# leodd/Lifted-Hybrid-Variational-Inference

Measured on AMD Instinct MI355X. Metric: lbp_sweeps_per_sec_10M_edge_hybrid_mrf, higher is better.
Workload: dtype f64

## Files before the change

### include/lhvi.h

```cpp
#ifndef LHVI_H
#define LHVI_H

#include <stddef.h>
#include <stdint.h>

#ifdef __cplusplus
extern "C" {
#endif

#define LHVI_ABI_VERSION 27
#define LHVI_MAX_ARITY 6

#define LHVI_OK 0
#define LHVI_E_ARG (-1)
#define LHVI_E_LAUNCH (-2)
#define LHVI_E_UNSUPPORTED (-3)
#define LHVI_E_NODEVICE (-4)
#define LHVI_E_NOT_PD (-5)

#define LHVI_POT_GENERIC 0
#define LHVI_POT_TABLE 1
#define LHVI_POT_GAUSSIAN 2
#define LHVI_POT_QUADRATIC 3
#define LHVI_POT_HYBRID_QUADRATIC 4
#define LHVI_POT_LINEAR_GAUSSIAN 5
#define LHVI_POT_X2 6
#define LHVI_POT_XY 7
#define LHVI_POT_MLN 8
#define LHVI_POT_MLN_HARD 9
#define LHVI_POT_IMAGE_NODE 10
#define LHVI_POT_IMAGE_EDGE 11

typedef struct lhvi_graph {
    int32_t V, F, E, nnz;
    const int32_t* fac_ptr;
    const int32_t* edge_var;
    const int32_t* edge_fac;
    const int32_t* edge_canon;
    const int32_t* var_ptr;
    const int32_t* var_edge;
    const double* edge_count;
    const int32_t* fac_pot;
    const double* var_value;
// ... 41 lines not shown
    const int32_t* seg;
    int32_t n_seg;
} lhvi_gabp_plan_t;
size_t lhvi_gabp_pull_workspace_bytes(const lhvi_graph_t* g);
int lhvi_gabp_pull(const lhvi_graph_t* g, const lhvi_pots_t* pots, const lhvi_gabp_plan_t* plan, const double* v_prev,
                   double* v_next, int first, void* stream);
int lhvi_gabp_run_pull(const lhvi_graph_t* g, const lhvi_pots_t* pots, const lhvi_gabp_plan_t* plan, double* f2v, double* v2f,
                       int iterations, void* ws, size_t ws_bytes, void* stream);

int lhvi_gabp_graph_create(const lhvi_graph_t* g, const lhvi_pots_t* pots, const lhvi_gabp_plan_t* plan, double* f2v, double* v2f,
                           double* mu_var, int iterations, void* ws, size_t ws_bytes, void** handle_out);
int lhvi_gabp_graph_launch(void* handle, void* stream);
int lhvi_gabp_graph_destroy(void* handle);

int lhvi_gabp_marginals(const lhvi_graph_t* g, const double* f2v, double* mu_var, void* stream);

size_t lhvi_log_likelihood_workspace_bytes(const lhvi_graph_t* g);
int lhvi_log_likelihood(const lhvi_graph_t* g, const lhvi_pots_t* pots, const double* x, double* out, void* ws, size_t ws_bytes,
                        void* stream);


#define LHVI_PBP_EP 1u
#define LHVI_PBP_EPBP_DISCRETE 2u
#define LHVI_PBP_SKIP_TERMS 16u
#define LHVI_PBP_LEAVE_ROOM 256u
#define LHVI_PBP_CQ 512u
#define LHVI_PBP_BOUNDARY_TOTALS 2048u
#define LHVI_PBP_NO_UNIQ 4096u
#define LHVI_PBP_V2F_RECORDS 8192u
#define LHVI_PBP_WIDE_PAIRS 16384u
#define LHVI_PBP_SHARE_CUS 32768u
#define LHVI_PBP_NO_GRID 128u
#define LHVI_PBP_FUSED_RECORDS16 131072u
#define LHVI_PBP_F2V_HEAVY 262144u
#define LHVI_PBP_F2V_SMALL 524288u
#define LHVI_PBP_F2V_PAIR 1048576u
#define LHVI_PBP_F2V_FAST 2097152u
#define LHVI_PBP_F2V_CQ 4194304u
#define LHVI_PBP_F2V_GENERIC 8388608u
#define LHVI_PBP_F2V_ALL (LHVI_PBP_F2V_HEAVY | LHVI_PBP_F2V_SMALL | LHVI_PBP_F2V_PAIR | LHVI_PBP_F2V_FAST | LHVI_PBP_F2V_CQ | LHVI_PBP_F2V_GENERIC)
#define LHVI_PBP_POW2_GROUPS 65536u

typedef struct lhvi_pbp {
    int32_t n;
    int32_t T;
    uint32_t flags;
    double var_threshold;
    double max_log_value;
    const double* particles;
    const double* old_particles;
    const int32_t* np;
    const uint8_t* uniq;
    const double* q;
    const int32_t* fast_edges;
    int32_t n_fast;
    const int32_t* generic_edges;
    int32_t n_generic;
    int32_t generic_pts_log2;
    const void* fast_desc;
    const void* heavy_desc;
    int32_t n_heavy;
    const void* light_desc;
    int32_t n_light;
    const int32_t* bslot;
    const int32_t* brow_ptr;
    const int64_t* brow_off;
// ... 400 lines not shown
```

### lifted-hybrid-variational-inference_amd/csrc/pbp.hip

```cpp
#include "common.hpp"
#include "potential.hpp"
#include "fastmath.hpp"
#include "cq.hpp"
#include "gk21.hpp"

namespace lhvi {

__device__ __forceinline__ double wave_sum(double v) { return dpp_wave_reduce(v, SumOp()); }
__device__ __forceinline__ double wave_max(double v) { return dpp_wave_reduce(v, MaxOp()); }
__device__ __forceinline__ int wave_sum_i(int v) {
#pragma unroll
    for (int off = 32; off > 0; off >>= 1) v += __shfl_xor(v, off);
    return v;
}

constexpr double PAD_LOG_TERM = -6.0e5;

__host__ __device__ __forceinline__ int var_first(const lhvi_pbp_t& s) { return s.var_hi > s.var_lo ? s.var_lo : 0; }
__host__ __device__ __forceinline__ int var_limit(const lhvi_graph_t& g, const lhvi_pbp_t& s) { return s.var_hi > s.var_lo ? s.var_hi : g.V; }

__device__ __forceinline__ double norm_pdf_std(double x, double mu, double sig) {
    const double u = (x - mu) / sig;
    return exp(-u * u * 0.5) / (2.506628274631 * sig);
}
// ... 197 lines not shown
    for (; k < deg; k += NW) {
        const int e = g.var_edge[lo + k];
        const double m = valid ? f2v[(int64_t)e * S + lane] : 0.0;
        acc += lifted ? m * g.edge_count[e] : m;
    }
    part[wid][lane] = acc;
    __syncthreads();
    double total = 0.0;
#pragma unroll
    for (int w = 0; w < NW; ++w) total += part[w][lane];
    const int d = g.var_dom[v];
    const double mu = s.q[2 * v], sd = sqrt_pos(s.q[2 * v + 1]), rsd = rcp_newton(sd);
    const double log_norm = log_pos(2.506628274631 * sd);
    const double x = valid ? s.particles[(int64_t)v * n + lane] : 0.0;
    const bool uq = valid && s.uniq[(int64_t)v * n + lane];
    const double logw = valid ? log_importance(g, s, v, d, x, mu, rsd, log_norm) : 0.0;
    const double rcnt = rcp_newton((double)__builtin_popcountll(__ballot(uq)));
    for (k = wid; k < deg; k += NW) {
        const int e = g.var_edge[lo + k];
        const double m = valid ? f2v[(int64_t)e * S + lane] : 0.0;
        const double res = (total - m) + logw;
        const double mean = wave_sum(uq ? res : 0.0) * rcnt;
        double shift = mean;
        if (__ballot(uq && (res - mean > s.max_log_value))) shift = wave_max(uq ? res : -__builtin_huge_val()) - s.max_log_value;
        if (valid) {
            v2f[(int64_t)e * n + lane] = res - shift;
            const int64_t halo = HALO ? s.halo_off[e] : -1;
            if (HALO && halo >= 0) s.halo_buf[halo + lane] = res - shift;
        }
    }
}

template <bool HALO>
__global__ void __launch_bounds__(BLOCK) pbp_v2f_narrow_kernel(lhvi_graph_t g, lhvi_pbp_t s, const double* __restrict__ f2v,
                                                              double* __restrict__ v2f) {
    const int lane = threadIdx.x & 63;
    const int64_t slot = ((int64_t)blockIdx.x * (BLOCK / WAVE) + (threadIdx.x >> 6)) * 16 + (lane >> 2);
    const int j = lane & 3;
    const int v = slot < s.n_v2f_narrow ? s.v2f_narrow[slot] : -1;
    const int n = s.n, S = s.n + s.T;
    const bool on = v >= 0 && is_hidden(g.var_value[v]);
    const int np = on ? s.np[v] : 0;
    const bool valid = j < np;
    const int lo = on ? g.var_ptr[v] : 0, deg = on ? g.var_ptr[v + 1] - lo : 0;
    const bool lifted = g.edge_count != nullptr;
    double total = 0.0;
    for (int k = 0; k < deg; ++k) {
        const int e = g.var_edge[lo + k];
        const double m = valid ? f2v[(int64_t)e * S + j] : 0.0;
        total += lifted ? m * g.edge_count[e] : m;
    }
    double logw = 0.0;
    bool uq = false;
    if (valid) {
        const int d = g.var_dom[v];
        const double sd = sqrt_pos(s.q[2 * v + 1]);
        logw = log_importance(g, s, v, d, s.particles[(int64_t)v * n + j], s.q[2 * v], rcp_newton(sd), log_pos(2.506628274631 * sd));
        uq = s.uniq[(int64_t)v * n + j] != 0;
    }
    auto quad_sum = [](double x) { x += dpp_move<0xb1>(x); return x + dpp_move<0x4e>(x); };
    auto quad_max = [](double x) { x = fmax(x, dpp_move<0xb1>(x)); return fmax(x, dpp_move<0x4e>(x)); };
    const double rcnt = rcp_newton(fmax(quad_sum(uq ? 1.0 : 0.0), 1.0));
    int maxdeg = deg;
#pragma unroll
    for (int off = 32; off > 0; off >>= 1) maxdeg = max(maxdeg, __shfl_xor(maxdeg, off));
    for (int k = 0; k < maxdeg; ++k) {
        const bool live = k < deg;
        const int e = live ? g.var_edge[lo + k] : 0;
        const double m = (live && valid) ? f2v[(int64_t)e * S + j] : 0.0;
        const double res = (total - m) + logw;
        const double mean = quad_sum(uq ? res : 0.0) * rcnt;
        const double mx = quad_max(uq ? res : -__builtin_huge_val());
        const double shift = (mx - mean > s.max_log_value) ? mx - s.max_log_value : mean;
        if (live && valid) {
            v2f[(int64_t)e * n + j] = res - shift;
            const int64_t halo = HALO ? s.halo_off[e] : -1;
            if (HALO && halo >= 0) s.halo_buf[halo + j] = res - shift;
        }
    }
}

template <int W, bool HALO>
__global__ void __launch_bounds__(BLOCK) pbp_v2f_packed_kernel(lhvi_graph_t g, lhvi_pbp_t s, const double* __restrict__ f2v,
                                                              double* __restrict__ v2f, const int32_t* __restrict__ list, int count) {
    constexpr int G = WAVE / W;
    const int lane = threadIdx.x & 63;
    const int64_t slot = ((int64_t)blockIdx.x * (BLOCK / WAVE) + (threadIdx.x >> 6)) * G + lane / W;
    const int j = lane % W;
    const int v = slot < count ? list[slot] : -1;
    const int n = s.n, S = s.n + s.T;
    const bool on = v >= 0 && is_hidden(g.var_value[v]);
    const int np = on ? s.np[v] : 0;
    const bool valid = j < np;
    const int lo = on ? g.var_ptr[v] : 0, deg = on ? g.var_ptr[v + 1] - lo : 0;
    const bool lifted = g.edge_count != nullptr;
    double total = 0.0;
    for (int k = 0; k < deg; ++k) {
        const int e = g.var_edge[lo + k];
        const double m = valid ? f2v[(int64_t)e * S + j] : 0.0;
        total += lifted ? m * g.edge_count[e] : m;
    }
    double logw = 0.0;
    bool uq = false;
    if (valid) {
        const int d = g.var_dom[v];
        const double sd = sqrt_pos(s.q[2 * v + 1]);
        logw = log_importance(g, s, v, d, s.particles[(int64_t)v * n + j], s.q[2 * v], rcp_newton(sd), log_pos(2.506628274631 * sd));
        uq = s.uniq[(int64_t)v * n + j] != 0;
    }
    auto group_sum = [&](double x) { return W == 16 ? dpp_move<0x15F>(dpp_row_reduce(x, SumOp())) : dpp_half_reduce(x, SumOp(), lane); };
    auto group_max = [&](double x) { return W == 16 ? dpp_row_reduce(x, MaxOp()) : dpp_half_reduce(x, MaxOp(), lane); };
    const uint64_t mine = (W == 16 ? 0xffffull : 0xffffffffull) << (lane / W * W);
    const double rcnt = rcp_newton(fmax((double)__builtin_popcountll(__ballot(uq) & mine), 1.0));
// ... 2124 lines not shown
                while (todo) {
                    const int k = __builtin_ctzll(todo);
                    const int klo = __builtin_amdgcn_readlane(xlo[h], k), khi = __builtin_amdgcn_readlane(xhi[h], k);
                    const uint64_t same = __ballot(xlo[h] == klo && xhi[h] == khi) & live;
                    dp |= same & (same - 1);
                    todo &= ~same;
                }
            }
            const int u = (lane < cn) && !((dp >> lane) & 1);
            if (lane < n) uniq[(int64_t)vv[h] * n + lane] = (uint8_t)u;
        }
    }
}

#ifndef LHVI_FUSED_WAVES
#define LHVI_FUSED_WAVES 4
#endif
constexpr int FUSED_CH = 8;
#ifndef LHVI_FUSED_NB
#define LHVI_FUSED_NB 2
#endif
#ifndef LHVI_FUSED64_WAVES
#define LHVI_FUSED64_WAVES 8
#endif
#ifndef LHVI_FUSED64_CH
#define LHVI_FUSED64_CH 4
#endif
#ifndef LHVI_FUSED64_PRE
#define LHVI_FUSED64_PRE 1
#endif
#ifndef LHVI_FUSED64_EARLY
#define LHVI_FUSED64_EARLY 1
#endif
#ifndef LHVI_FUSED64_LATE_TABLE
#define LHVI_FUSED64_LATE_TABLE 1
#endif
constexpr int FUSED_CH64 = LHVI_FUSED64_CH;
constexpr int FUSED64_HASH_BITS = 12;
template <int W, int PW, bool EP, bool R16>
__global__ void __launch_bounds__(BLOCK) __attribute__((amdgpu_waves_per_eu(W == 64 ? (PW == 32 || EP ? LHVI_FUSED_WAVES : LHVI_FUSED64_WAVES) : LHVI_FUSED_WAVES, 8)))
pbp_var_fused_kernel(lhvi_graph_t g, lhvi_pbp_t s, const double* __restrict__ f2v, double* __restrict__ v2f, double* __restrict__ eta,
                     double* __restrict__ q, const int64_t* __restrict__ gid, uint64_t seed, uint32_t iteration,
                     double* __restrict__ out, uint8_t* __restrict__ uniq, const int32_t* __restrict__ list, int count) {
    __shared__ LogRec sh_log[LOG_TAB_N];
    __shared__ uint8_t sh_owner[W == 64 ? (BLOCK / WAVE) << FUSED64_HASH_BITS : 1];
    constexpr bool LATE_TABLE = W == 64 && LHVI_FUSED64_LATE_TABLE != 0;
    double tab_inv = 0.0, tab_log = 0.0;
    if constexpr (LATE_TABLE) {
        if (threadIdx.x < LOG_TAB_N) { tab_inv = LOG_TAB[2 * threadIdx.x]; tab_log = LOG_TAB[2 * threadIdx.x + 1]; }
    } else {
        load_log_table(sh_log);
        __syncthreads();
    }
    constexpr int G = WAVE / W, SL = W / PW;
    const int lane = threadIdx.x & 63;
    const int wave = W == 64 ? __builtin_amdgcn_readfirstlane(threadIdx.x >> 6) : (int)(threadIdx.x >> 6);
    const int64_t slot = ((int64_t)blockIdx.x * (BLOCK / WAVE) + wave) * G + lane / W;
    const int j = lane % W;
    const bool on = slot < count;
    const int32_t* rec = list + (R16 ? 16 : 8) * (on ? slot : 0);
    int4 ra, rb;
    int2 rc = make_int2(0, 0);
    int e_rec = 0;
    if (R16) {
        const int4* r4 = reinterpret_cast<const int4*>(rec);
        ra = r4[0]; rb = r4[1]; rc = reinterpret_cast<const int2*>(rec)[4];
        e_rec = rec[10 + min(lane % W, 5)];
    } else {
        ra = make_int4(rec[0], rec[1], rec[2], rec[3]); rb = make_int4(rec[4], rec[5], rec[6], rec[7]);
    }
    const int v = on ? ra.x : 0;
    const int deg = on ? ra.y : 0, gb = ra.z, T = on ? ra.w : 0;
    const double dlo = __hiloint2double(rb.y, rb.x), dhi = __hiloint2double(rb.w, rb.z);
    const int n = s.n, S = s.n + s.T;
    const int np = on ? (R16 ? rc.x : s.np[v]) : 0;
    const bool valid = j < np;
    const int lo = on ? (R16 ? rc.y : g.var_ptr[v]) : 0;
    const bool lifted = g.edge_count != nullptr;
    const double q0 = on ? s.q[2 * v] : 0.0, q1 = on ? s.q[2 * v + 1] : 1.0;
    int maxdeg = deg;
#pragma unroll
    for (int off = 32; off >= W; off >>= 1) maxdeg = max(maxdeg, __shfl_xor(maxdeg, off));
    constexpr int CH = W == 64 ? FUSED_CH64 : FUSED_CH;
    static_assert(W >= CH && CH % SL == 0, "lane j of a group holds edge j of the chunk");
    static_assert(W < 64 || R16, "the one-variable-per-wavefront form reads sixteen-word records");
    const int first_lane = lane / W * W;
    const int nch = (maxdeg + CH - 1) / CH;
    int my_e = 0, held = -1;
    auto hold_chunk = [&](int c) {
        if (c == held) return;
// ... 648 lines not shown
    hipLaunchKernelGGL(pbp_belief_kernel, dim3(grid_for((int64_t)nq * npts)), dim3(BLOCK), 0, as_stream(stream), *g, *pots, *s,
                       v2f, nq, qvar, npts, x, out);
    return check_launch();
}

int lhvi_pbp_map_brent(const lhvi_graph_t* g, const lhvi_pots_t* pots, const lhvi_pbp_t* s, const double* v2f, int64_t nq,
                       const int32_t* row_var, const int64_t* qptr, const int32_t* qedge, const double* qmult, double xtol,
                       int32_t maxfun, double* xout, double* fout, int32_t* nfev, void* stream) {
    if (int rc = validate_pbp(g, s)) return rc;
    if (!pots || !v2f || nq < 0 || maxfun < 1 || !(xtol > 0.0)) return LHVI_E_ARG;
    if (nq == 0) return LHVI_OK;
    if (!row_var || !xout || !g->dom_lo || !g->dom_hi || !g->dom_val) return LHVI_E_ARG;
    if (qptr && (!qedge || !qmult)) return LHVI_E_ARG;
    QueryRows rows{row_var, qptr, qedge, qmult};
    hipLaunchKernelGGL(pbp_map_brent_kernel, dim3(grid_for(nq)), dim3(BLOCK), 0, as_stream(stream), *g, *pots, *s, v2f, nq, rows,
                       row_var, xtol / 3.0, maxfun, xout, fout, nfev);
    return check_launch();
}

int lhvi_pbp_var_fused(const lhvi_graph_t* g, const lhvi_pbp_t* s, const double* f2v, double* v2f, double* eta, double* q,
                       const int64_t* var_gid, uint64_t seed, uint32_t iteration, double* particles_out, uint8_t* uniq_out,
                       const int32_t* desc, int32_t n16, int32_t n32_t32, int32_t n32_t64, void* stream) {
    if (int rc = validate_pbp(g, s)) return rc;
    if (!f2v || !v2f || !eta || !q || !particles_out || !uniq_out || !s->uniq || !s->q || !g->dom_lo || !g->dom_hi || !g->dom_val) return LHVI_E_ARG;
    if (n16 < 0 || n32_t32 < 0 || n32_t64 < 0 || s->n > 32 || s->bslot || s->var_hi > s->var_lo || particles_out == s->particles) return LHVI_E_ARG;
    if ((int64_t)n16 + n32_t32 + n32_t64 == 0) return LHVI_OK;
    if (!desc) return LHVI_E_ARG;
    hipStream_t st = as_stream(stream);
    const bool ep = (s->flags & LHVI_PBP_EP) != 0;
#define LHVI_FUSED(W, PW, list, cnt)                                                                                                  \
    if ((cnt) > 0) {                                                                                                                  \
        const dim3 grid(grid_for(((int64_t)(cnt) + WAVE / (W) - 1) / (WAVE / (W)) * WAVE));                                          \
        if (ep && r16) hipLaunchKernelGGL((pbp_var_fused_kernel<W, PW, true, true>), grid, dim3(BLOCK), 0, st, *g, *s, f2v, v2f, eta, q, var_gid, \
                                   seed, iteration, particles_out, uniq_out, list, cnt);                                             \
        else if (ep) hipLaunchKernelGGL((pbp_var_fused_kernel<W, PW, true, false>), grid, dim3(BLOCK), 0, st, *g, *s, f2v, v2f, eta, q, var_gid, \
                                   seed, iteration, particles_out, uniq_out, list, cnt);                                             \
        else if (r16) hipLaunchKernelGGL((pbp_var_fused_kernel<W, PW, false, true>), grid, dim3(BLOCK), 0, st, *g, *s, f2v, v2f, eta, q, var_gid,   \
                                seed, iteration, particles_out, uniq_out, list, cnt);                                                \
        else hipLaunchKernelGGL((pbp_var_fused_kernel<W, PW, false, false>), grid, dim3(BLOCK), 0, st, *g, *s, f2v, v2f, eta, q, var_gid,   \
                                seed, iteration, particles_out, uniq_out, list, cnt);                                                \
    }
    const bool r16 = (s->flags & LHVI_PBP_FUSED_RECORDS16) != 0;
    const int64_t rw = r16 ? 16 : 8;
    LHVI_FUSED(16, 16, desc, n16)
    LHVI_FUSED(32, 16, desc + rw * (int64_t)n16, n32_t32)
    LHVI_FUSED(32, 32, desc + rw * ((int64_t)n16 + n32_t32), n32_t64)
#undef LHVI_FUSED
    return check_launch();
}

int lhvi_pbp_var_fused64(const lhvi_graph_t* g, const lhvi_pbp_t* s, const double* f2v, double* v2f, double* eta, double* q,
                         const int64_t* var_gid, uint64_t seed, uint32_t iteration, double* particles_out, uint8_t* uniq_out,
                         const int32_t* desc, int32_t n64_t32, int32_t n64_t64, void* stream) {
    if (int rc = validate_pbp(g, s)) return rc;
    if (!f2v || !v2f || !eta || !q || !particles_out || !uniq_out || !s->uniq || !s->q || !g->dom_lo || !g->dom_hi || !g->dom_val) return LHVI_E_ARG;
    if (n64_t32 < 0 || n64_t64 < 0 || s->n <= 32 || s->n > 64 || s->bslot || s->var_hi > s->var_lo || particles_out == s->particles) return LHVI_E_ARG;
    if ((int64_t)n64_t32 + n64_t64 == 0) return LHVI_OK;
    if (!desc) return LHVI_E_ARG;
    hipStream_t st = as_stream(stream);
    const bool ep = (s->flags & LHVI_PBP_EP) != 0;
#define LHVI_FUSED64(PW, list, cnt)                                                                                                   \
    if ((cnt) > 0) {                                                                                                                  \
        const dim3 grid(grid_for((int64_t)(cnt) * WAVE));                                                                             \
        if (ep) hipLaunchKernelGGL((pbp_var_fused_kernel<64, PW, true, true>), grid, dim3(BLOCK), 0, st, *g, *s, f2v, v2f, eta, q, var_gid, \
                                   seed, iteration, particles_out, uniq_out, list, cnt);                                             \
        else hipLaunchKernelGGL((pbp_var_fused_kernel<64, PW, false, true>), grid, dim3(BLOCK), 0, st, *g, *s, f2v, v2f, eta, q, var_gid,   \
                                seed, iteration, particles_out, uniq_out, list, cnt);                                                \
    }
    LHVI_FUSED64(16, desc, n64_t32)
    LHVI_FUSED64(32, desc + 16 * (int64_t)n64_t32, n64_t64)
#undef LHVI_FUSED64
    return check_launch();
}

int lhvi_pbp_quad(const lhvi_graph_t* g, const lhvi_pots_t* pots, const lhvi_pbp_t* s, const double* v2f, int64_t nq,
                  const int32_t* row_var, const int64_t* qptr, const int32_t* qedge, const double* qmult, const double* lo,
                  const double* hi, double epsabs, double epsrel, double* z, double* abserr, int32_t* status, void* stream) {
    if (int rc = validate_pbp(g, s)) return rc;
    if (!pots || !v2f || nq < 0 || !(epsabs >= 0.0) || !(epsrel >= 0.0)) return LHVI_E_ARG;
    if (nq == 0) return LHVI_OK;
    if (!row_var || !lo || !hi || !z) return LHVI_E_ARG;
    if (qptr && (!qedge || !qmult)) return LHVI_E_ARG;
    QueryRows rows{row_var, qptr, qedge, qmult};
    hipLaunchKernelGGL(pbp_quad_kernel, dim3(grid_for(nq)), dim3(BLOCK), 0, as_stream(stream), *g, *pots, *s, v2f, nq, rows, row_var,
                       lo, hi, epsabs, epsrel, z, abserr, status);
    return check_launch();
}

int lhvi_pbp_kl(const lhvi_graph_t* g, const lhvi_pots_t* pots, const lhvi_pbp_t* s, const double* v2f, int64_t nq,
                const int32_t* row_var, const int64_t* qptr, const int32_t* qedge, const double* qmult, const double* logz,
                int32_t Kp, const double* wp, const double* mup, const double* varp, const double* a, const double* b,
                double epsabs, double epsrel, double* kl, double* abserr, int32_t* status, int32_t* neval, void* stream) {
    if (int rc = validate_pbp(g, s)) return rc;
    if (!pots || !v2f || nq < 1 || nq > 0x7fffffff || Kp < 1 || !(epsabs >= 0.0) || !(epsrel >= 0.0)) return LHVI_E_ARG;
    if (!row_var || !logz || !wp || !mup || !varp || !a || !b || !kl) return LHVI_E_ARG;
    if (g->V < 1 || !g->dom_lo || !g->dom_hi || !g->dom_val) return LHVI_E_ARG;
    if (qptr && (!qedge || !qmult)) return LHVI_E_ARG;
    QueryRows rows{row_var, qptr, qedge, qmult};
    hipLaunchKernelGGL(pbp_kl_kernel, dim3((unsigned)nq), dim3(WAVE), 0, as_stream(stream), *g, *pots, *s, v2f, rows, row_var, logz,
                       Kp, wp, mup, varp, a, b, epsabs, epsrel, kl, abserr, status, neval);
// ... 5 lines not shown
```

### lifted-hybrid-variational-inference_amd/lhvi/_abi.py

```python
from __future__ import annotations

import ctypes as C
import os

import numpy as np

_HERE = os.path.dirname(os.path.abspath(__file__))
LIB_PATH = os.environ.get('LHVI_LIB') or os.path.join(os.path.dirname(_HERE), 'csrc', 'liblhvi.so')

c_i32p = C.c_void_p
c_f64p = C.c_void_p


class LhviError(RuntimeError):
    pass


class GraphStruct(C.Structure):
    _fields_ = [
        ('V', C.c_int32), ('F', C.c_int32), ('E', C.c_int32), ('nnz', C.c_int32),
        ('fac_ptr', C.c_void_p), ('edge_var', C.c_void_p), ('edge_fac', C.c_void_p), ('edge_canon', C.c_void_p),
        ('var_ptr', C.c_void_p), ('var_edge', C.c_void_p), ('edge_count', C.c_void_p), ('fac_pot', C.c_void_p),
        ('var_value', C.c_void_p), ('var_dom', C.c_void_p), ('var_mult', C.c_void_p), ('fac_mult', C.c_void_p),
        ('D', C.c_int32),
# ... 35 lines not shown
        ('halo_off', C.c_void_p), ('halo_buf', C.c_void_p),
    ]


class ViStruct(C.Structure):
    _fields_ = [
        ('K', C.c_int32), ('T', C.c_int32), ('Dmax', C.c_int32), ('quirks', C.c_int32),
        ('gh_x', C.c_void_p), ('gh_w', C.c_void_p), ('w', C.c_void_p), ('eta_c', C.c_void_p), ('eta_d', C.c_void_p),
        ('obs_var', C.c_void_p), ('var_N', C.c_void_p),
        ('fac_list', C.c_void_p), ('n_cc', C.c_int32), ('n_grp3', C.c_int32), ('n_grp6', C.c_int32), ('n_rest3', C.c_int32),
        ('n_rest6', C.c_int32), ('n_tiny', C.c_int32), ('tiny_par_words', C.c_int32), ('edge_axis', C.c_void_p),
    ]


class ViOptStruct(C.Structure):
    _fields_ = [(n, C.c_void_p) for n in ('w_tau', 'w', 'eta_c', 'tau_d', 'eta_d', 'm_w', 's_w', 'm_c', 's_c', 'm_d', 's_d',
                                          'g_w', 'g_c', 'g_d', 'fe')] + \
               [(n, C.c_double) for n in ('lr', 'b1', 'b2', 'eps', 'var_min')] + [('t', C.c_int32)]


PBP_EP = 1
PBP_EPBP_DISCRETE = 2
PBP_SKIP_TERMS = 16
PBP_NO_GRID = 128
PBP_LEAVE_ROOM = 256
PBP_BOUNDARY_TOTALS = 2048
PBP_CQ = 512
PBP_NO_UNIQ = 4096
PBP_V2F_RECORDS = 8192
PBP_WIDE_PAIRS = 16384
PBP_SHARE_CUS = 32768
PBP_POW2_GROUPS = 65536
PBP_FUSED_RECORDS16 = 131072
PBP_F2V_HEAVY = 262144
PBP_F2V_SMALL = 524288
PBP_F2V_PAIR = 1048576
PBP_F2V_FAST = 2097152
PBP_F2V_CQ = 4194304
PBP_F2V_GENERIC = 8388608
PBP_F2V_ALL = PBP_F2V_HEAVY | PBP_F2V_SMALL | PBP_F2V_PAIR | PBP_F2V_FAST | PBP_F2V_CQ | PBP_F2V_GENERIC
ABI_VERSION = 27
PBP_DESC_BYTES = 128
COLOR_HASH, COLOR_SORT = 0, 1
HUB_DEGREE = 64
VI_GROUP_SLOTS, VI_GROUP_COMP, VI_TINY_NODES, VI_TINY_K, VI_TINY_PAR = 24, 48, 32, 2, 3072

class MwsStruct(C.Structure):
    _fields_ = [('T', C.c_int32), ('max_flips', C.c_int32), ('epsilon', C.c_double), ('noise_std', C.c_double),
                ('seed', C.c_uint64), ('try_id', C.c_void_p), ('disc', C.c_void_p), ('n_disc', C.c_int32),
                ('num', C.c_void_p), ('n_num', C.c_int32), ('fac_class', C.c_void_p), ('x', C.c_void_p), ('best_x', C.c_void_p),
                ('cur_score', C.c_void_p), ('best_score', C.c_void_p), ('status', C.c_void_p), ('err_flip', C.c_void_p),
                ('rec_score', C.c_void_p), ('rec_zero', C.c_void_p), ('rec_ticks', C.c_void_p)] + \
               [(n, C.c_void_p) for n in ('rp_init', 'rp_clause', 'rp_walk', 'rp_walk_k', 'rp_noise', 'rp_post', 'out_score',
                                          'out_unsat', 'out_winner', 'out_accept', 'out_val')]


class ExactStruct(C.Structure):
    _fields_ = [('Nd', C.c_int32), ('Nc', C.c_int32), ('M', C.c_int64), ('dstates', C.c_void_p), ('dstride', C.c_void_p),
                ('n_quad', C.c_int32), ('quad_ptr', C.c_void_p), ('quad_desc', C.c_void_p), ('quad_par', C.c_void_p),
                ('n_tab', C.c_int32), ('tab_ptr', C.c_void_p), ('tab_desc', C.c_void_p), ('tab_par', C.c_void_p)]


class GibbsStruct(C.Structure):
    _fields_ = [('ex', ExactStruct), ('dstate_off', C.c_void_p), ('vt_ptr', C.c_void_p), ('vt_fac', C.c_void_p),
                ('vh_ptr', C.c_void_p), ('vh_fac', C.c_void_p), ('n_hyb', C.c_int32), ('hyb_quad', C.c_void_p),
                ('hyb_off', C.c_void_p), ('table_doubles', C.c_int32), ('max_states', C.c_int32), ('table_scratch', C.c_void_p),
                ('disc_block_its', C.c_int32), ('num_burnin', C.c_int32), ('num_samples', C.c_int32), ('seed', C.c_uint64)]


E_NOT_PD = -5
EXACT_MAX_NC = 64
GAUSS_EXACT_NB = 64
GAUSS_CHAIN_MAX_BLOCK = 128

# ... 343 lines not shown
```

### lifted-hybrid-variational-inference_amd/lhvi/pbp.py

```python
from __future__ import annotations

import os
from math import e, log, sqrt

import numpy as np

from . import _abi, pbp_plan, pbp_query
from .flat import flatten

_F2V_LONG = _abi.PBP_F2V_HEAVY | _abi.PBP_F2V_SMALL
_F2V_SHORT = _abi.PBP_F2V_PAIR | _abi.PBP_F2V_FAST | _abi.PBP_F2V_CQ | _abi.PBP_F2V_GENERIC
F2V_SCHEDULES = {
    'one': (('main', _abi.PBP_F2V_ALL, 0, False),),
    'timed': (('main', _F2V_LONG, 0, True), ('main', _F2V_SHORT, 0, False)),
    'overlap': (('side', _F2V_SHORT, 0, False), ('main', _F2V_LONG, _abi.PBP_SHARE_CUS, True)),
}


def _stream(st):
    return _abi.stream_ptr() if st is None else st


class _ParticleSweep:
    var_threshold = 3
# ... 49 lines not shown
        self._static_rows = False
        self.var_lists = plan.on(_abi.upload(plan.host), dg.zeros(plan.n_prop_partial, 2) if plan.n_prop_partial else None)
        for name, value in self.var_lists.named().items():
            setattr(self, name, value)
        self._has_f_side = 'f' in sides
        self.f2v_lists = pbp_plan.F2vLists.empty(torch.zeros(1, dtype=torch.int32, device=dg.device))
        if self._has_f_side:
            cls = torch.zeros(max(flat.E, 1), dtype=torch.uint8, device=dg.device)
            _abi.check(_abi.lib().lhvi_pbp_classify(dg.g, dg.p, self._struct(), _abi.ptr(cls), _abi.stream_ptr()))
            self.f2v_lists = pbp_plan.f_side_plan(
                cls[:flat.E], flat, self.np_host, describe=self._describe,
                describe_cq=lambda edges: self._describe(edges, 'lhvi_pbp_describe_cq', 2 * _abi.PBP_DESC_BYTES),
                skip=None if edge_skip is None else _abi.to_dev(np.ascontiguousarray(edge_skip, dtype=bool)),
                key=None if edge_key is None else _abi.to_dev(np.ascontiguousarray(edge_key, dtype=np.int32)),
                paired_light=self.paired_light, small_f2v=self.small_f2v, long_grid_min_edges=self.long_grid_min_edges)
        for name, value in self.f2v_lists.named().items():
            setattr(self, name, value)

    def _describe(self, edges, entry='lhvi_pbp_describe', nbytes=_abi.PBP_DESC_BYTES):
        torch = _abi.require_gpu()
        k = int(edges.numel())
        desc = torch.empty(k * nbytes, dtype=torch.uint8, device=edges.device)
        _abi.check(getattr(_abi.lib(), entry)(self.dg.g, self.dg.p, self._struct(), _abi.ptr(edges), k, _abi.ptr(desc), _abi.stream_ptr()))
        return desc

    def _plan_options(self):
        env = os.environ.get
        return pbp_plan.PlanOptions(
            sampler_on_device=self.sampler == 'device', listed_proposal=self.listed_proposal, listed_resample=self.listed_resample,
            sliced_proposal=self.sliced_proposal, prop_slice=self.prop_slice, packed_v2f=self.packed_v2f,
            v2f_records=env('LHVI_PBP_V2F_REC', '1') != '0',
            fused=self.fused_var_kernel and env('LHVI_PBP_FUSED', '1') != '0',
            fused_max_particles=int(env('LHVI_PBP_FUSED_MAX', self.fused_max_particles)),
            fused_records16=env('LHVI_PBP_FUSED_REC16', '1') != '0')

    def _struct(self, var_range=None, leave_room=False):
        s = _abi.PbpStruct()
        s.n, s.T, s.flags = self.n, self.T, self.flags | (_abi.PBP_LEAVE_ROOM if leave_room else 0)
        s.var_threshold, s.max_log_value = float(self.var_threshold), float(self.max_log_value)
        s.particles, s.old_particles = _abi.ptr(self.particles), _abi.ptr(self.old_particles)
        s.uniq, s.q = _abi.ptr(self.uniq), _abi.ptr(self.q_dev)
        self.f2v_lists.install(s)
        if var_range is None:
            self.var_lists.install(s, self.listed_proposal)
        else:
            self.var_lists.install_range(s, *var_range)
        s.f2v_ticket = _abi.ptr(self.f2v_ticket) if self.dynamic_f2v else None
        return s

    def _launch_init(self, s, st=None):
        _abi.check(_abi.lib().lhvi_pbp_init(self.dg.g, s, _abi.ptr(self.eta), _abi.ptr(self.q_dev), _abi.ptr(self.f2v), _abi.ptr(self.v2f),
                                            _stream(st)))

    def _launch_v2f(self, s, st=None):
        _abi.check(_abi.lib().lhvi_pbp_v2f(self.dg.g, s, _abi.ptr(self.f2v), _abi.ptr(self.v2f), _stream(st)))

    def _launch_proposal(self, s, st=None):
        _abi.check(_abi.lib().lhvi_pbp_proposal(self.dg.g, s, _abi.ptr(self.f2v), _abi.ptr(self.eta), _abi.ptr(self.q_dev), _stream(st)))

    def _launch_proposal_partial(self, s, ph, st=None):
        _abi.check(_abi.lib().lhvi_pbp_proposal_partial(self.dg.g, s, _abi.ptr(self.f2v), _abi.ptr(self.eta), _abi.ptr(ph), _stream(st)))

    def _launch_proposal_finish(self, s, ph, st=None):
        _abi.check(_abi.lib().lhvi_pbp_proposal_finish(self.dg.g, s, _abi.ptr(ph), _abi.ptr(self.q_dev), _stream(st)))

    def _launch_draw(self, s, st=None):
        _abi.check(_abi.lib().lhvi_pbp_resample_uniq(self.dg.g, s, _abi.ptr(self.var_gid), int(self.seed), int(self._draws - 1),
# ... 47 lines not shown
            by_list = rest_only or (listed and self._static_rows)
            if rest_only:
                L.install_rest(s, 'sampler')
            elif by_list:
                L.install_sampler(s)
            if not by_list or s.n_resample_vars:
                self._launch_draw(s)
            if listed and not self._static_rows:
                if L.static_idx is not None:
                    self.old_particles.index_copy_(0, L.static_idx, self.particles.index_select(0, L.static_idx))
                self._static_rows = True
            return
        k = self._draws
        self._draws += 1
        if callable(self.sampler):
            self._install(self.sampler(k, self.flat, self.q_dev.cpu().numpy()))
        else:
            self._install(self._host_draw())
        _abi.check(_abi.lib().lhvi_pbp_uniq(self.dg.g, self.n, _abi.ptr(self.particles), _abi.ptr(L.np_dev), _abi.ptr(self.uniq),
                                            _abi.stream_ptr()))
        self._views, self._batched = {}, {}

    def _run_sweeps(self, iteration):
        self._launch_init(self._struct())
        self._generate_sample()
        for i in range(iteration):
            self.sweep(last=(i == iteration - 1))
        self._views, self._batched = {}, {}

    def sweep(self, last=False, f2v_events=None):
        L, st = self.var_lists, _abi.stream_ptr()
        if not last and L.fused is not None and self._static_rows and self.sampler == 'device':
            s = self._struct()
            self._launch_fused(s, st)
            L.install_rest(s, 'v2f')
            self._launch_v2f(s, st)
            L.install_rest(s, 'proposal')
            self._launch_proposal(s, st)
            self._generate_sample(rest_only=True)
            self._launch_f2v(self._struct(), f2v_events, st)
            return
        self._launch_v2f(self._struct(), st)
        if last:
            self._batched = {}
        else:
            self._launch_proposal(self._struct(), st)
            self._generate_sample()
            self._launch_f2v(self._struct(), f2v_events, st)

    def _f2v_schedule(self, timed=False):
        want = os.environ.get('LHVI_PBP_OVERLAP')
        if (self.overlap_f2v or want == '1') and want != '0' and self.n_heavy >= self.overlap_min_heavy:
            return 'overlap'
        return 'timed' if timed else 'one'

    def _call_f2v(self, s, out=None, st=None):
        _abi.check(_abi.lib().lhvi_pbp_f2v(self.dg.g, self.dg.p, s, _abi.ptr(self.v2f), _abi.ptr(self.f2v if out is None else out),
                                           _stream(st)))

    def _launch_f2v(self, s, f2v_events=None, st=None):
        if not self._has_f_side:
            raise _abi.LhviError('this state was set up for the v -> f half only (sides="v")')
        st = _stream(st)
        calls = F2V_SCHEDULES[self._f2v_schedule(bool(f2v_events))]
        side = any(stream == 'side' for stream, _, _, _ in calls)
        if side:
            torch = _abi.require_gpu()
            main = torch.cuda.current_stream()
            if self._side is None:
# ... 815 lines not shown
```

### lifted-hybrid-variational-inference_amd/lhvi/pbp_plan.py

```python
from __future__ import annotations

from collections import namedtuple

import numpy as np

from . import _abi

V2F_CLASSES = ('wide', 'narrow', 'hub', 'mid16', 'mid32')

PlanOptions = namedtuple('PlanOptions', 'sampler_on_device listed_proposal listed_resample sliced_proposal prop_slice packed_v2f '
                                        'v2f_records fused fused_max_particles fused_records16')

class V2fLists(namedtuple('V2fLists', 'wide n_wide narrow n_narrow hub n_hub mid16 n_mid16 mid32 n_mid32', defaults=(None, 0) * 5)):

    def install(self, s):
        for name in V2F_CLASSES:
            setattr(s, 'v2f_' + name, _abi.ptr(getattr(self, name)))
            setattr(s, 'n_v2f_' + name, getattr(self, 'n_' + name))

    def named(self, prefix):
        return {prefix + name: getattr(self, name) for name in V2F_CLASSES}

    def on(self, dev, prefix):
        return self._replace(**{name: dev[prefix + name] for name in V2F_CLASSES})


class FusedLists(namedtuple('FusedLists', 'counts counts64 desc desc64 v2f_rest prop_desc_rest n_prop_rest resample_rest n_resample_rest')):

    def __getitem__(self, key):
        return getattr(self, key) if isinstance(key, str) else tuple.__getitem__(self, key)

    def named(self):
        return {'fused_desc': self.desc, 'fused64_desc': self.desc64, 'prop_desc_rest': self.prop_desc_rest,
                'resample_rest': self.resample_rest, **self.v2f_rest.named('v2f_rest_')}

    def on(self, dev):
        return self._replace(desc=dev['fused_desc'], desc64=dev.get('fused64_desc'), prop_desc_rest=dev['prop_desc_rest'],
                             resample_rest=dev['resample_rest'], v2f_rest=self.v2f_rest.on(dev, 'v2f_rest_'))


class VarLists(namedtuple('VarLists', 'np_dev resample_vars n_resample_vars static_idx prop_desc n_prop_desc prop_hub n_prop_hub prop_partial '
                                      'v2f fused')):

    def named(self):
        return dict(np_dev=self.np_dev, resample_vars=self.resample_vars, n_prop_desc=self.n_prop_desc, prop_hub=self.prop_hub,
                    n_prop_hub=self.n_prop_hub, v2f_lists=self.v2f, _fused=self.fused)

    def install(self, s, proposal_records=True):
        s.np = _abi.ptr(self.np_dev)
        if self.v2f is not None:
            self.v2f.install(s)
        if proposal_records and self.prop_desc is not None:
            s.prop_desc, s.n_prop_desc = _abi.ptr(self.prop_desc), self.n_prop_desc
            if self.prop_hub is not None:
                s.prop_hub, s.n_prop_hub, s.prop_partial = _abi.ptr(self.prop_hub), self.n_prop_hub, _abi.ptr(self.prop_partial)

    def install_range(self, s, lo, hi):
        s.np = _abi.ptr(self.np_dev)
        s.prop_desc, s.n_prop_desc = None, 0
        s.prop_hub, s.n_prop_hub, s.prop_partial = None, 0, None
# ... 109 lines not shown
        ph[:, 0], ph[:, 1], ph[:, 2] = pv[hubs], first, nsl
        pd = np.concatenate([sl, np.delete(pd, hubs, axis=0)])
        host['prop_hub'], n_prop_hub, n_prop_partial = ph, int(hubs.size), int(owner.size)
    host['prop_desc'] = np.ascontiguousarray(pd) if pv.size else None
    hidden_v = np.flatnonzero(flat.var_hidden)
    if owned is not None:
        hidden_v = hidden_v[hidden_v < owned]
    flags, v2f, fused = 0, None, None
    if opts.packed_v2f and hidden_v.size:
        v2f = v2f_split(flat, np_host, hidden_v, opts.v2f_records)
        if v2f.n_wide == hidden_v.size:
            v2f = None
    if v2f is not None:
        host.update(v2f.named('v2f_'))
        flags |= _abi.PBP_V2F_RECORDS if opts.v2f_records else 0
    fz = (pdeg <= min(64, opts.prop_slice)) & (pT <= 64) & (n <= min(64, opts.fused_max_particles))
    if opts.fused and owned is None and opts.sampler_on_device and opts.listed_proposal and opts.listed_resample \
            and v2f is not None and fz.any():
        k16 = fz & (n <= 16) & (pT <= 32)
        k32a = fz & (n <= 32) & ~k16 & (pT <= 32)
        k32b = fz & (n <= 32) & ~k16 & ~k32a
        k64a = fz & (n > 32) & (pT <= 32)
        k64b = fz & (n > 32) & ~k64a
        fd64 = np.zeros((pv.size, 16), dtype=np.int32)
        fd64[:, 0], fd64[:, 1], fd64[:, 2], fd64[:, 3] = pv, pdeg, flat.dom_ptr[pdom], pT
        fd64[:, 4:6], fd64[:, 6:8] = _double_words(flat.dom_lo[pdom]), _double_words(flat.dom_hi[pdom])
        fd64[:, 8], fd64[:, 9] = np_host[pv], flat.var_ptr[pv]
        fd64[:, 10:] = first_edges(flat, pv, 6, clamp=False)
        fd = fd64 if opts.fused_records16 else fd64[:, :8]
        flags |= _abi.PBP_FUSED_RECORDS16 if opts.fused_records16 else 0
        fused_var = np.zeros(flat.V, dtype=bool)
        fused_var[pv[fz]] = True
        keep, rkeep = ~fused_var[pd[:, 0]], ~fused_var[rr[:, 0]]
        fused = FusedLists(counts=(int(k16.sum()), int(k32a.sum()), int(k32b.sum())), counts64=(int(k64a.sum()), int(k64b.sum())),
                           desc=_or_zero_row(np.concatenate([fd[k16], fd[k32a], fd[k32b]])),
                           desc64=np.ascontiguousarray(np.concatenate([fd64[k64a], fd64[k64b]])) if k64a.any() or k64b.any() else None,
                           v2f_rest=v2f_split(flat, np_host, hidden_v[~fused_var[hidden_v]], opts.v2f_records),
                           prop_desc_rest=_or_zero_row(pd[keep]), n_prop_rest=int(keep.sum()),
                           resample_rest=_or_zero_row(rr[rkeep]), n_resample_rest=int(rkeep.sum()))
        host.update({k: a for k, a in fused.named().items() if a is not None})
    return VarSidePlan(host=host, flags=flags, np_host=np_host, T=T, n_prop_desc=int(pd.shape[0]), n_prop_hub=n_prop_hub,
                       n_prop_partial=n_prop_partial, v2f=v2f, fused=fused)


F2vSplit = namedtuple('F2vSplit', 'heavy small16 small32 light rest heavy_terms heavy_grid_terms')


def f2v_split(words, small_f2v, long_grid_min_edges):
    base = (words[:, 4] == 1) & (words[:, 6] != 4)
    small16 = small32 = base.new_zeros(base.shape)
    if small_f2v:
        small16 = base & (words[:, 7] <= 16) & (words[:, 8] <= 16)
        small32 = base & ~small16 & (words[:, 7] <= 32) & (words[:, 8] <= 32)
    small = small16 | small32
    on_recurrence = (words[:, 15] == 1) & (words[:, 7] >= 24) & (words[:, 9] <= 128) & (words[:, 8] <= 128)
    two_rounds = words[:, 8] + words[:, 9] <= 128
    if int((on_recurrence & ~two_rounds & ~small).sum().item()) < long_grid_min_edges:
        on_recurrence = two_rounds
    heavy = (base & (words[:, 7] <= 64) & (two_rounds | on_recurrence)) | small
    hw = words[heavy].long()
    heavy_terms = int(((hw[:, 8] + hw[:, 9]) * hw[:, 7]).sum().item())
    on_grid = (hw[:, 15] == 1) & (hw[:, 9] <= 128) & ((hw[:, 7] >= 24) | small[heavy])
    heavy_grid_terms = int((hw[:, 9] * hw[:, 7])[on_grid].sum().item())
    light = ~heavy & (words[:, 14] != 0)
    return F2vSplit(heavy, small16, small32, light, ~heavy & ~light, heavy_terms, heavy_grid_terms)


def pair_records(light_words, E, key=None):
    import torch
    light = light_words.view(torch.uint8).view(-1, 128)
    dev = light.device
    w = light.view(torch.int32).view(-1, 32).long()
# ... 147 lines not shown
```

Baseline: 70.53.

## Fold narrow v2f kernel into fused64 var kernel launch as spread front blocks

The separate narrow-variable v2f kernel is merged into the fused64 variable kernel. Extra blocks are spread through the grid at power-of-two strides and run the narrow v2f body, while the remaining blocks run the fused work with a remapped block index. This removes one kernel launch and its tail and lets the narrow v2f work overlap with fused work. In exchange, the fused kernel carries the narrow body's code and register use. The path is enabled only when no other v2f classes remain and fused64 variables exist.

```diff
diff --git a/include/lhvi.h b/include/lhvi.h
--- a/include/lhvi.h
+++ b/include/lhvi.h
@@ -8,7 +8,7 @@
 extern "C" {
 #endif
 
-#define LHVI_ABI_VERSION 27
+#define LHVI_ABI_VERSION 28
 #define LHVI_MAX_ARITY 6
 
 #define LHVI_OK 0
@@ -116,6 +116,7 @@
 #define LHVI_PBP_SHARE_CUS 32768u
 #define LHVI_PBP_NO_GRID 128u
 #define LHVI_PBP_FUSED_RECORDS16 131072u
+#define LHVI_PBP_FUSED_V2F_NARROW 1024u
 #define LHVI_PBP_F2V_HEAVY 262144u
 #define LHVI_PBP_F2V_SMALL 524288u
 #define LHVI_PBP_F2V_PAIR 1048576u
diff --git a/lifted-hybrid-variational-inference_amd/csrc/pbp.hip b/lifted-hybrid-variational-inference_amd/csrc/pbp.hip
--- a/lifted-hybrid-variational-inference_amd/csrc/pbp.hip
+++ b/lifted-hybrid-variational-inference_amd/csrc/pbp.hip
@@ -253,10 +253,10 @@
 }
 
 template <bool HALO>
-__global__ void __launch_bounds__(BLOCK) pbp_v2f_narrow_kernel(lhvi_graph_t g, lhvi_pbp_t s, const double* __restrict__ f2v,
-                                                              double* __restrict__ v2f) {
+__device__ __forceinline__ void v2f_narrow_body(const lhvi_graph_t& g, const lhvi_pbp_t& s, const double* __restrict__ f2v,
+                                                double* __restrict__ v2f, unsigned block) {
     const int lane = threadIdx.x & 63;
-    const int64_t slot = ((int64_t)blockIdx.x * (BLOCK / WAVE) + (threadIdx.x >> 6)) * 16 + (lane >> 2);
+    const int64_t slot = ((int64_t)block * (BLOCK / WAVE) + (threadIdx.x >> 6)) * 16 + (lane >> 2);
     const int j = lane & 3;
     const int v = slot < s.n_v2f_narrow ? s.v2f_narrow[slot] : -1;
     const int n = s.n, S = s.n + s.T;
@@ -300,6 +300,12 @@
         }
     }
 }
+template <bool HALO>
+__global__ void __launch_bounds__(BLOCK) pbp_v2f_narrow_kernel(lhvi_graph_t g, lhvi_pbp_t s, const double* __restrict__ f2v,
+                                                              double* __restrict__ v2f) {
+    v2f_narrow_body<HALO>(g, s, f2v, v2f, blockIdx.x);
+}
+static inline int64_t v2f_narrow_blocks(int64_t count) { return (count + 16 * (BLOCK / WAVE) - 1) / (16 * (BLOCK / WAVE)); }
 
 template <int W, bool HALO>
 __global__ void __launch_bounds__(BLOCK) pbp_v2f_packed_kernel(lhvi_graph_t g, lhvi_pbp_t s, const double* __restrict__ f2v,
@@ -2490,6 +2496,9 @@
 #ifndef LHVI_FUSED64_EARLY
 #define LHVI_FUSED64_EARLY 1
 #endif
+#ifndef LHVI_FUSED64_NARROW_SPREAD
+#define LHVI_FUSED64_NARROW_SPREAD 1
+#endif
 #ifndef LHVI_FUSED64_LATE_TABLE
 #define LHVI_FUSED64_LATE_TABLE 1
 #endif
@@ -2499,7 +2508,14 @@
 __global__ void __launch_bounds__(BLOCK) __attribute__((amdgpu_waves_per_eu(W == 64 ? (PW == 32 || EP ? LHVI_FUSED_WAVES : LHVI_FUSED64_WAVES) : LHVI_FUSED_WAVES, 8)))
 pbp_var_fused_kernel(lhvi_graph_t g, lhvi_pbp_t s, const double* __restrict__ f2v, double* __restrict__ v2f, double* __restrict__ eta,
                      double* __restrict__ q, const int64_t* __restrict__ gid, uint64_t seed, uint32_t iteration,
-                     double* __restrict__ out, uint8_t* __restrict__ uniq, const int32_t* __restrict__ list, int count) {
+                     double* __restrict__ out, uint8_t* __restrict__ uniq, const int32_t* __restrict__ list, int count, unsigned front,
+                     unsigned front_shift) {
+    unsigned block = blockIdx.x;
+    if constexpr (W == 64) {
+        const unsigned q = blockIdx.x >> front_shift;
+        if ((blockIdx.x & ((1u << front_shift) - 1u)) == 0 && q < front) { v2f_narrow_body<false>(g, s, f2v, v2f, q); return; }
+        block = blockIdx.x - min(front, q + 1);
+    }
     __shared__ LogRec sh_log[LOG_TAB_N];
     __shared__ uint8_t sh_owner[W == 64 ? (BLOCK / WAVE) << FUSED64_HASH_BITS : 1];
     constexpr bool LATE_TABLE = W == 64 && LHVI_FUSED64_LATE_TABLE != 0;
@@ -2513,7 +2529,7 @@
     constexpr int G = WAVE / W, SL = W / PW;
     const int lane = threadIdx.x & 63;
     const int wave = W == 64 ? __builtin_amdgcn_readfirstlane(threadIdx.x >> 6) : (int)(threadIdx.x >> 6);
-    const int64_t slot = ((int64_t)blockIdx.x * (BLOCK / WAVE) + wave) * G + lane / W;
+    const int64_t slot = ((int64_t)block * (BLOCK / WAVE) + wave) * G + lane / W;
     const int j = lane % W;
     const bool on = slot < count;
     const int32_t* rec = list + (R16 ? 16 : 8) * (on ? slot : 0);
@@ -3228,13 +3244,13 @@
     if ((cnt) > 0) {                                                                                                                  \
         const dim3 grid(grid_for(((int64_t)(cnt) + WAVE / (W) - 1) / (WAVE / (W)) * WAVE));                                          \
         if (ep && r16) hipLaunchKernelGGL((pbp_var_fused_kernel<W, PW, true, true>), grid, dim3(BLOCK), 0, st, *g, *s, f2v, v2f, eta, q, var_gid, \
-                                   seed, iteration, particles_out, uniq_out, list, cnt);                                             \
+                                   seed, iteration, particles_out, uniq_out, list, cnt, 0u, 0u);                                      \
         else if (ep) hipLaunchKernelGGL((pbp_var_fused_kernel<W, PW, true, false>), grid, dim3(BLOCK), 0, st, *g, *s, f2v, v2f, eta, q, var_gid, \
-                                   seed, iteration, particles_out, uniq_out, list, cnt);                                             \
+                                   seed, iteration, particles_out, uniq_out, list, cnt, 0u, 0u);                                      \
         else if (r16) hipLaunchKernelGGL((pbp_var_fused_kernel<W, PW, false, true>), grid, dim3(BLOCK), 0, st, *g, *s, f2v, v2f, eta, q, var_gid,   \
-                                seed, iteration, particles_out, uniq_out, list, cnt);                                                \
+                                seed, iteration, particles_out, uniq_out, list, cnt, 0u, 0u);                                         \
         else hipLaunchKernelGGL((pbp_var_fused_kernel<W, PW, false, false>), grid, dim3(BLOCK), 0, st, *g, *s, f2v, v2f, eta, q, var_gid,   \
-                                seed, iteration, particles_out, uniq_out, list, cnt);                                                \
+                                seed, iteration, particles_out, uniq_out, list, cnt, 0u, 0u);                                         \
     }
     const bool r16 = (s->flags & LHVI_PBP_FUSED_RECORDS16) != 0;
     const int64_t rw = r16 ? 16 : 8;
@@ -3251,17 +3267,25 @@
     if (int rc = validate_pbp(g, s)) return rc;
     if (!f2v || !v2f || !eta || !q || !particles_out || !uniq_out || !s->uniq || !s->q || !g->dom_lo || !g->dom_hi || !g->dom_val) return LHVI_E_ARG;
     if (n64_t32 < 0 || n64_t64 < 0 || s->n <= 32 || s->n > 64 || s->bslot || s->var_hi > s->var_lo || particles_out == s->particles) return LHVI_E_ARG;
-    if ((int64_t)n64_t32 + n64_t64 == 0) return LHVI_OK;
+    if ((int64_t)n64_t32 + n64_t64 == 0) return (s->flags & LHVI_PBP_FUSED_V2F_NARROW) ? LHVI_E_ARG : LHVI_OK;
     if (!desc) return LHVI_E_ARG;
     hipStream_t st = as_stream(stream);
     const bool ep = (s->flags & LHVI_PBP_EP) != 0;
+    unsigned front = 0, shift = 0;
+    if (s->flags & LHVI_PBP_FUSED_V2F_NARROW) {
+        if (!s->v2f_narrow || s->n_v2f_narrow < 0 || s->halo_off) return LHVI_E_ARG;
+        front = (unsigned)v2f_narrow_blocks(s->n_v2f_narrow);
+    }
 #define LHVI_FUSED64(PW, list, cnt)                                                                                                   \
     if ((cnt) > 0) {                                                                                                                  \
-        const dim3 grid(grid_for((int64_t)(cnt) * WAVE));                                                                             \
+        const dim3 grid(grid_for((int64_t)(cnt) * WAVE) + front);                                                                     \
+             \
+        for (shift = 0; LHVI_FUSED64_NARROW_SPREAD && front > 0 && ((uint64_t)front << (shift + 1)) <= grid.x; ++shift) {}            \
         if (ep) hipLaunchKernelGGL((pbp_var_fused_kernel<64, PW, true, true>), grid, dim3(BLOCK), 0, st, *g, *s, f2v, v2f, eta, q, var_gid, \
-                                   seed, iteration, particles_out, uniq_out, list, cnt);                                             \
+                                   seed, iteration, particles_out, uniq_out, list, cnt, front, shift);                                \
         else hipLaunchKernelGGL((pbp_var_fused_kernel<64, PW, false, true>), grid, dim3(BLOCK), 0, st, *g, *s, f2v, v2f, eta, q, var_gid,   \
-                                seed, iteration, particles_out, uniq_out, list, cnt);                                                \
+                                seed, iteration, particles_out, uniq_out, list, cnt, front, shift);                                   \
+        front = 0; shift = 0;                                                                                                         \
     }
     LHVI_FUSED64(16, desc, n64_t32)
     LHVI_FUSED64(32, desc + 16 * (int64_t)n64_t32, n64_t64)
diff --git a/lifted-hybrid-variational-inference_amd/lhvi/_abi.py b/lifted-hybrid-variational-inference_amd/lhvi/_abi.py
--- a/lifted-hybrid-variational-inference_amd/lhvi/_abi.py
+++ b/lifted-hybrid-variational-inference_amd/lhvi/_abi.py
@@ -91,6 +91,7 @@
 PBP_SHARE_CUS = 32768
 PBP_POW2_GROUPS = 65536
 PBP_FUSED_RECORDS16 = 131072
+PBP_FUSED_V2F_NARROW = 1024
 PBP_F2V_HEAVY = 262144
 PBP_F2V_SMALL = 524288
 PBP_F2V_PAIR = 1048576
@@ -98,7 +99,7 @@
 PBP_F2V_CQ = 4194304
 PBP_F2V_GENERIC = 8388608
 PBP_F2V_ALL = PBP_F2V_HEAVY | PBP_F2V_SMALL | PBP_F2V_PAIR | PBP_F2V_FAST | PBP_F2V_CQ | PBP_F2V_GENERIC
-ABI_VERSION = 27
+ABI_VERSION = 28
 PBP_DESC_BYTES = 128
 COLOR_HASH, COLOR_SORT = 0, 1
 HUB_DEGREE = 64
diff --git a/lifted-hybrid-variational-inference_amd/lhvi/pbp.py b/lifted-hybrid-variational-inference_amd/lhvi/pbp.py
--- a/lifted-hybrid-variational-inference_amd/lhvi/pbp.py
+++ b/lifted-hybrid-variational-inference_amd/lhvi/pbp.py
@@ -105,7 +105,8 @@
             v2f_records=env('LHVI_PBP_V2F_REC', '1') != '0',
             fused=self.fused_var_kernel and env('LHVI_PBP_FUSED', '1') != '0',
             fused_max_particles=int(env('LHVI_PBP_FUSED_MAX', self.fused_max_particles)),
-            fused_records16=env('LHVI_PBP_FUSED_REC16', '1') != '0')
+            fused_records16=env('LHVI_PBP_FUSED_REC16', '1') != '0',
+            fused_narrow=env('LHVI_PBP_FUSED_NARROW', '1') != '0')
 
     def _struct(self, var_range=None, leave_room=False):
         s = _abi.PbpStruct()
@@ -219,9 +220,15 @@
         L, st = self.var_lists, _abi.stream_ptr()
         if not last and L.fused is not None and self._static_rows and self.sampler == 'device':
             s = self._struct()
-            self._launch_fused(s, st)
-            L.install_rest(s, 'v2f')
-            self._launch_v2f(s, st)
+            if L.fused.narrow_in_fused64:
+                L.install_rest(s, 'v2f')
+                s.flags |= _abi.PBP_FUSED_V2F_NARROW
+                self._launch_fused(s, st)
+                s.flags &= ~_abi.PBP_FUSED_V2F_NARROW
+            else:
+                self._launch_fused(s, st)
+                L.install_rest(s, 'v2f')
+                self._launch_v2f(s, st)
             L.install_rest(s, 'proposal')
             self._launch_proposal(s, st)
             self._generate_sample(rest_only=True)
diff --git a/lifted-hybrid-variational-inference_amd/lhvi/pbp_plan.py b/lifted-hybrid-variational-inference_amd/lhvi/pbp_plan.py
--- a/lifted-hybrid-variational-inference_amd/lhvi/pbp_plan.py
+++ b/lifted-hybrid-variational-inference_amd/lhvi/pbp_plan.py
@@ -9,7 +9,7 @@
 V2F_CLASSES = ('wide', 'narrow', 'hub', 'mid16', 'mid32')
 
 PlanOptions = namedtuple('PlanOptions', 'sampler_on_device listed_proposal listed_resample sliced_proposal prop_slice packed_v2f '
-                                        'v2f_records fused fused_max_particles fused_records16')
+                                        'v2f_records fused fused_max_particles fused_records16 fused_narrow', defaults=(True,))
 
 class V2fLists(namedtuple('V2fLists', 'wide n_wide narrow n_narrow hub n_hub mid16 n_mid16 mid32 n_mid32', defaults=(None, 0) * 5)):
 
@@ -25,7 +25,8 @@
         return self._replace(**{name: dev[prefix + name] for name in V2F_CLASSES})
 
 
-class FusedLists(namedtuple('FusedLists', 'counts counts64 desc desc64 v2f_rest prop_desc_rest n_prop_rest resample_rest n_resample_rest')):
+class FusedLists(namedtuple('FusedLists', 'counts counts64 desc desc64 v2f_rest prop_desc_rest n_prop_rest resample_rest n_resample_rest '
+                                          'narrow_in_fused64', defaults=(False,))):
 
     def __getitem__(self, key):
         return getattr(self, key) if isinstance(key, str) else tuple.__getitem__(self, key)
@@ -201,12 +202,15 @@
         fused_var = np.zeros(flat.V, dtype=bool)
         fused_var[pv[fz]] = True
         keep, rkeep = ~fused_var[pd[:, 0]], ~fused_var[rr[:, 0]]
+        v2f_rest = v2f_split(flat, np_host, hidden_v[~fused_var[hidden_v]], opts.v2f_records)
         fused = FusedLists(counts=(int(k16.sum()), int(k32a.sum()), int(k32b.sum())), counts64=(int(k64a.sum()), int(k64b.sum())),
                            desc=_or_zero_row(np.concatenate([fd[k16], fd[k32a], fd[k32b]])),
                            desc64=np.ascontiguousarray(np.concatenate([fd64[k64a], fd64[k64b]])) if k64a.any() or k64b.any() else None,
-                           v2f_rest=v2f_split(flat, np_host, hidden_v[~fused_var[hidden_v]], opts.v2f_records),
+                           v2f_rest=v2f_rest,
                            prop_desc_rest=_or_zero_row(pd[keep]), n_prop_rest=int(keep.sum()),
-                           resample_rest=_or_zero_row(rr[rkeep]), n_resample_rest=int(rkeep.sum()))
+                           resample_rest=_or_zero_row(rr[rkeep]), n_resample_rest=int(rkeep.sum()),
+                           narrow_in_fused64=bool(opts.fused_narrow and (k64a.any() or k64b.any())
+                                                  and not (v2f_rest.n_wide or v2f_rest.n_hub or v2f_rest.n_mid16 or v2f_rest.n_mid32)))
         host.update({k: a for k, a in fused.named().items() if a is not None})
     return VarSidePlan(host=host, flags=flags, np_host=np_host, T=T, n_prop_desc=int(pd.shape[0]), n_prop_hub=n_prop_hub,
                        n_prop_partial=n_prop_partial, v2f=v2f, fused=fused)
```

New measurement: 62.93. 10.8% lower.
